# BurntSushi/rust-snappy

Hardware: NVIDIA H100
Metric: uncompressed GB/s, raw 64KB-block compress+decompress round trip (higher is better)
Workload: dtype u8

## Files before the change

### rust-snappy_b200/csrc/k2_decompress.cuh

```cuda
#pragma once
#include "common.cuh"

namespace sbk {

static const uint32_t K2_SMEM_PER_WARP = 256;

SB_DEVICE uint32_t k2_read_header(const uint8_t* in, uint32_t n, uint64_t* value) {
    uint64_t v = 0;
    unsigned shift = 0;
    for (uint32_t i = 0; i < n; i++) {
        if (shift >= 64) return 0;
        uint32_t b = in[i];
        if (b < 0x80) { *value = v | ((uint64_t)b << shift); return i + 1; }
        v |= (uint64_t)(b & 0x7F) << shift;
        shift += 7;
    }
    return 0;
}

template <bool kHeader = true>
SB_DEVICE uint32_t k2_decode_stream(const uint8_t* in, uint32_t n, uint8_t* dst, uint64_t cap,
                                    sb_error* st, uint32_t* out_len, uint32_t* elems) {
    const unsigned lane = lane_id();
    uint64_t dn64 = cap;
    uint32_t hl = 0;
    if constexpr (kHeader) {
        if (n == 0) { if (lane == 0) set_status(st, SB_EMPTY, 0, 0, 0); return SB_EMPTY; }
        dn64 = 0;
        hl = k2_read_header(in, n, &dn64);
        if (hl == 0) { if (lane == 0) set_status(st, SB_HEADER, 0, 0, 0); return SB_HEADER; }
        if (dn64 > kMaxInput) { if (lane == 0) set_status(st, SB_TOO_BIG, dn64, kMaxInput, 0); return SB_TOO_BIG; }
        if (dn64 > cap) { if (lane == 0) set_status(st, SB_BUFFER_TOO_SMALL, cap, dn64, 0); return SB_BUFFER_TOO_SMALL; }
    }

    const uint8_t* src = in + hl;
    const uint8_t* in_end = in + n;
    const uint32_t sn = n - hl, dn = (uint32_t)dn64;
    uint32_t s = 0, d = 0;

    while (s < sn) {
#include "k2_window.inc"
        const bool is_start = ((M >> lane) & 1u) && valid;
        const unsigned last = 31 - clz(M);

        uint32_t olen = (is_start && !spill) ? (uint32_t)len : 0u;
        uint32_t incl = olen;
#pragma unroll
        for (int k = 1; k < 32; k <<= 1) {
            const uint32_t t = shfl_up(incl, k);
            if (lane >= (unsigned)k) incl += t;
        }
        const uint32_t opos = incl - olen;
        const uint32_t win_out = shfl(incl, 31);
        const uint64_t de = (uint64_t)d + opos;
        const uint64_t sa = (uint64_t)s + lane + 1;

        const bool sure = (rem >= 40) && (dn - d >= win_out) &&
                          !any(is_start && (spill || (kind != 0 && (off == 0 || off > d + opos))));
        if (!sure) {
            uint32_t ecode = 0; uint64_t ea = 0, eb = 0, ec = 0;
            if (is_start) {
                if (kind == 0) {
                    uint64_t sp = sa;
                    if ((tag >> 2) >= 60) {
                        if (sa + 4 > sn) { ecode = SB_LITERAL; ea = 4; eb = sn - sa; ec = dn - de; }
                        sp = sa + (hdr - 1);
                    }
                    if (!ecode && (sn - sp < len || dn - de < len)) {
                        ecode = SB_LITERAL; ea = len; eb = sn - sp; ec = dn - de;
                    }
                } else {
                    const unsigned nb = hdr - 1;
                    if (sa + 4 > sn) {
                        if (nb == 1) { if (sa >= sn) { ecode = SB_COPY_READ; ea = 1; eb = sn - sa; } }
                        else if (nb == 2) { if (sa + 1 >= sn) { ecode = SB_COPY_READ; ea = 2; eb = sn - sa; } }
                        else { ecode = SB_COPY_READ; ea = 4; eb = sn - sa; }
                    }
                    if (!ecode && (off == 0 || de < off)) { ecode = SB_OFFSET; ea = off; eb = de; }
                    if (!ecode && de + len > dn) { ecode = SB_COPY_WRITE; ea = len; eb = dn - de; }
                }
            }
            const uint32_t emask = ballot(ecode != 0);
            if (emask) {
                const unsigned first = ffs(emask) - 1;
                if (lane == first) set_status(st, ecode, ea, eb, ec);
                return shfl(ecode, first);
            }
        }

        {
            const unsigned own = 31 - clz(M & (0xFFFFFFFFu >> (31 - lane)));
            const uint32_t pk = shfl((opos << 8) | (hdr << 4) | (kind << 1) | (spill ? 1u : 0u), own);
            const unsigned ohdr = (pk >> 4) & 0xFu;
            if (valid && (pk & 7u) == 0 && lane >= own + ohdr)
                dst[d + (pk >> 8) + (lane - own - ohdr)] = (uint8_t)tag;
        }
        syncwarp();

        {
            uint8_t* const wout = dst + d;
            const uint32_t cpk = opos | ((uint32_t)len << 12);
            const bool is_copy = is_start && kind != 0;
            const bool indep = is_copy && (uint32_t)len <= 32 && off >= opos + (uint32_t)len;
            const uint32_t im = ballot(indep);
            if (im) {
                const uint32_t ilen = indep ? (uint32_t)len : 0u;
                uint32_t cincl = ilen;
#pragma unroll
                for (int k = 1; k < 32; k <<= 1) {
                    const uint32_t t2 = shfl_up(cincl, k);
                    if (lane >= (unsigned)k) cincl += t2;
                }
                const uint32_t cpos = cincl - ilen, ctot = shfl(cincl, 31);
                if (indep) {
                    const uint32_t rk = popc(im & ((1u << lane) - 1u));
                    elems[rk * 2] = cpk | (cpos << 20);
                    elems[rk * 2 + 1] = off;
                }
                syncwarp();
                for (uint32_t base = 0; base < ctot; base += 64) {
                    uint32_t dsto[2], srco[2];
                    uint8_t v[2];
                    bool on[2];
#pragma unroll
                    for (int q = 0; q < 2; q++) {
                        const uint32_t lo = base + 32 * q;
                        const uint32_t bit = (indep && cpos >= lo && cpos < lo + 32) ? 1u << (cpos - lo) : 0u;
                        const uint32_t Bm = reduce_or(bit);
                        const uint32_t before = popc(ballot(indep && cpos < lo));
                        const uint32_t t = lo + lane;
                        on[q] = t < ctot;
                        const uint32_t rk = before + popc(Bm & (0xFFFFFFFFu >> (31 - lane))) - 1;
                        const uint32_t e0 = on[q] ? elems[rk * 2] : 0u, e1 = on[q] ? elems[rk * 2 + 1] : 0u;
                        dsto[q] = (e0 & 0xFFFu) + (t - (e0 >> 20));
                        srco[q] = e1;
                    }
#pragma unroll
                    for (int q = 0; q < 2; q++) v[q] = on[q] ? wout[(int64_t)dsto[q] - (int64_t)srco[q]] : (uint8_t)0;
#pragma unroll
                    for (int q = 0; q < 2; q++) if (on[q]) wout[dsto[q]] = v[q];
                }
            }
            syncwarp();
            uint32_t cm = ballot(is_copy && !indep);
            while (cm) {
                const unsigned j = ffs(cm) - 1;
                cm &= cm - 1;
                const uint32_t pk1 = shfl(cpk, j), coff = shfl(off, j);
                const uint32_t clen = pk1 >> 12;
                uint8_t* out = wout + (pk1 & 0xFFFu);
                if (coff >= clen || clen <= 32) {
                    if (lane < clen) out[lane] = out[(int64_t)(coff >= clen || lane < coff ? lane : lane % coff) - (int64_t)coff];
                    if (clen > 32 && lane + 32 < clen) out[lane + 32] = out[(int64_t)lane + 32 - (int64_t)coff];
                } else {
                    const uint8_t* from = out - coff;
                    for (uint32_t k = lane; k < clen; k += 32) out[k] = from[k % coff];
                }
                syncwarp();
            }
        }

        const uint32_t lpk = shfl((uint32_t)(spill ? 1u : 0u) | (hdr << 1), last);
        if (lpk & 1u) {
            const uint32_t llen = shfl((uint32_t)len, last);
            const uint32_t lsrc = s + last + (lpk >> 1);
            warp_copy(dst + d + win_out, src + lsrc, llen);
            syncwarp();
            s = lsrc + llen;
            d += win_out + llen;
        } else {
            s += shfl(E, 0);
            d += win_out;
        }
    }
    if (d != dn) {
        if (lane == 0) set_status(st, SB_HEADER_MISMATCH, dn, d, 0);
        return SB_HEADER_MISMATCH;
    }
    if (lane == 0) { set_status(st, SB_OK, 0, 0, 0); if (out_len) *out_len = (uint32_t)dn; }
    return SB_OK;
}

SB_DEVICE void k2_decompress_body(const BatchDesc& b) {
    const unsigned warps_per_block = block_dim() >> 5;
    uint32_t* elems = (uint32_t*)smem() + warp_id() * 64;
    const uint64_t nwarps = (uint64_t)grid_dim() * warps_per_block;
    for (uint64_t u = (uint64_t)block_idx() * warps_per_block + warp_id(); u < b.count; u += nwarps) {
        const uint32_t i = (uint32_t)u;
        if (b.out_lens && lane_id() == 0) b.out_lens[i] = 0;
        k2_decode_stream(unit_in(b, i), unit_in_len(b, i), unit_out(b, i), unit_out_cap(b, i),
                         b.statuses ? &b.statuses[i] : nullptr, b.out_lens ? &b.out_lens[i] : nullptr, elems);
    }
}

}
```

### rust-snappy_b200/csrc/k2_window.inc

```
const uintptr_t A = (uintptr_t)(src + s);
const unsigned mis = (unsigned)(A & 3u);
uint32_t word = 0;
if (lane < 10) {
    const uint8_t* wp = (const uint8_t*)(A - mis) + 4 * lane;
    if (wp >= in && wp + 4 <= in_end) {
        word = *(const uint32_t*)wp;
    } else {
        for (int k = 0; k < 4; k++)
            if (wp + k >= in && wp + k < in_end) word |= (uint32_t)wp[k] << (8 * k);
    }
}
const unsigned bi = mis + lane;
const uint32_t lo = shfl(word, bi >> 2), hi = shfl(word, (bi >> 2) + 1);
const unsigned sh = (bi & 3u) * 8;
const uint32_t tag = funnel_r(lo, hi, sh) & 0xFFu;
const uint32_t next4 = sh == 24 ? hi : funnel_r(lo, hi, sh + 8);
const uint32_t rem = sn - s;
const bool valid = lane < rem;

const unsigned kind = tag & 3u;
unsigned hdr;
uint64_t len;
uint32_t off = 0;
if (kind == 0) {
    const unsigned L = tag >> 2;
    if (L < 60) { hdr = 1; len = L + 1; }
    else {
        const unsigned nb = L - 59;
        hdr = 1 + nb;
        len = (uint64_t)(nb == 4 ? next4 : (next4 & ((1u << (8 * nb)) - 1))) + 1;
    }
} else if (kind == 1) {
    hdr = 2; len = 4 + ((tag >> 2) & 7u); off = ((tag >> 5) << 8) | (next4 & 0xFFu);
} else if (kind == 2) {
    hdr = 3; len = 1 + (tag >> 2); off = next4 & 0xFFFFu;
} else {
    hdr = 5; len = 1 + (tag >> 2); off = next4;
}
const bool spill = valid && kind == 0 && (uint64_t)lane + hdr + len > 32;
uint32_t E = !valid ? 64u : spill ? 64u : (uint32_t)(lane + hdr + (kind == 0 ? (uint32_t)len : 0u));

uint32_t M = 1u << lane;
#pragma unroll
for (int r = 0; r < 4; r++) {
    const uint32_t M2 = shfl(M, E & 31u), E2 = shfl(E, E & 31u);
    if (E < 32) { M |= M2; E = E2; }
}
M = shfl(M, 0);
```

### rust-snappy_b200/csrc/simt.h

```cpp
#pragma once
#include <stdint.h>
#include <stddef.h>

#if defined(SB_EMU)
#ifndef SB_EMU_PRIMITIVES
#error "SB_EMU builds must include tests/emu/simt_emu.h first (it defines the warp primitives)"
#endif
namespace sbk {
SB_DEVICE void prefetch_l2(const void*) {}
}
#else

#include <cuda_runtime.h>

#define SB_DEVICE __device__ __forceinline__
#define SB_DEVICE_NOINLINE __device__ __noinline__
#define SB_FULL 0xFFFFFFFFu

namespace sbk {

SB_DEVICE unsigned lane_id() { return threadIdx.x & 31u; }
SB_DEVICE unsigned warp_id() { return threadIdx.x >> 5; }
SB_DEVICE unsigned thread_idx() { return threadIdx.x; }
SB_DEVICE unsigned block_dim() { return blockDim.x; }
SB_DEVICE unsigned block_idx() { return blockIdx.x; }
SB_DEVICE unsigned grid_dim() { return gridDim.x; }

SB_DEVICE uint32_t shfl(uint32_t v, unsigned src) { return __shfl_sync(SB_FULL, v, src); }
SB_DEVICE int shfl(int v, unsigned src) { return __shfl_sync(SB_FULL, v, src); }
SB_DEVICE uint64_t shfl(uint64_t v, unsigned src) { return __shfl_sync(SB_FULL, v, src); }
SB_DEVICE uint32_t shfl_up(uint32_t v, unsigned d) { return __shfl_up_sync(SB_FULL, v, d); }
SB_DEVICE uint32_t shfl_down(uint32_t v, unsigned d) { return __shfl_down_sync(SB_FULL, v, d); }
SB_DEVICE uint32_t shfl_xor(uint32_t v, unsigned m) { return __shfl_xor_sync(SB_FULL, v, m); }
SB_DEVICE uint32_t ballot(bool p) { return __ballot_sync(SB_FULL, p); }
SB_DEVICE bool any(bool p) { return __any_sync(SB_FULL, p); }
SB_DEVICE bool all(bool p) { return __all_sync(SB_FULL, p); }
SB_DEVICE uint32_t match_any(uint32_t v) { return __match_any_sync(SB_FULL, v); }
SB_DEVICE void syncwarp() { __syncwarp(); }
SB_DEVICE void syncthreads() { __syncthreads(); }
SB_DEVICE void bar_sync(unsigned id, unsigned nthreads) {
    asm volatile("bar.sync %0, %1;" ::"r"(id), "r"(nthreads) : "memory");
}
SB_DEVICE void bar_arrive(unsigned id, unsigned nthreads) {
    asm volatile("bar.arrive %0, %1;" ::"r"(id), "r"(nthreads) : "memory");
}

SB_DEVICE int popc(uint32_t v) { return __popc(v); }
SB_DEVICE int ffs(uint32_t v) { return __ffs(v); }
SB_DEVICE int clz(uint32_t v) { return __clz(v); }
SB_DEVICE int ffsll(uint64_t v) { return __ffsll((long long)v); }
SB_DEVICE uint32_t funnel_r(uint32_t lo, uint32_t hi, unsigned sh) { return __funnelshift_r(lo, hi, sh); }
SB_DEVICE uint32_t byte_perm(uint32_t a, uint32_t b, uint32_t s) { return __byte_perm(a, b, s); }

SB_DEVICE uint32_t atomic_add(uint32_t* p, uint32_t v) { return atomicAdd(p, v); }
SB_DEVICE unsigned long long atomic_add(unsigned long long* p, unsigned long long v) { return atomicAdd(p, v); }
SB_DEVICE uint32_t atomic_min(uint32_t* p, uint32_t v) { return atomicMin(p, v); }
SB_DEVICE void threadfence() { __threadfence(); }
SB_DEVICE void threadfence_block() { __threadfence_block(); }
SB_DEVICE uint32_t reduce_or(uint32_t v) { return __reduce_or_sync(SB_FULL, v); }
SB_DEVICE uint32_t reduce_add(uint32_t v) { return __reduce_add_sync(SB_FULL, v); }
SB_DEVICE uint32_t reduce_max(uint32_t v) { return __reduce_max_sync(SB_FULL, v); }
SB_DEVICE void spin() { __nanosleep(32); }
SB_DEVICE void spin_long() { __nanosleep(1500); }
SB_DEVICE uint32_t ld_volatile(const uint32_t* p) { return *(const volatile uint32_t*)p; }
SB_DEVICE void st_volatile(uint32_t* p, uint32_t v) { *(volatile uint32_t*)p = v; }
SB_DEVICE uint64_t ld_volatile64(const uint64_t* p) { return *(const volatile uint64_t*)p; }
SB_DEVICE void prefetch_l2(const void* p) { asm volatile("prefetch.global.L2 [%0];" :: "l"(p)); }

SB_DEVICE uint32_t ldg32(const void* p) { return __ldg((const uint32_t*)p); }
SB_DEVICE uint4 ldg128(const void* p) { return __ldg((const uint4*)p); }
SB_DEVICE uint8_t ldg8(const void* p) { return __ldg((const uint8_t*)p); }
SB_DEVICE void stcs128(void* p, uint4 v) { __stcs((uint4*)p, v); }

SB_DEVICE void mbar_init(uint64_t* bar, unsigned count) {
    asm volatile("mbarrier.init.shared::cta.b64 [%0], %1;" ::"r"((uint32_t)__cvta_generic_to_shared(bar)), "r"(count) : "memory");
}
SB_DEVICE void mbar_arrive(uint64_t* bar) {
    asm volatile("mbarrier.arrive.shared::cta.b64 _, [%0];" ::"r"((uint32_t)__cvta_generic_to_shared(bar)) : "memory");
}
SB_DEVICE bool mbar_try_wait(uint64_t* bar, unsigned parity, unsigned hint_ns) {
    uint32_t done;
    asm volatile("{ .reg .pred p; mbarrier.try_wait.parity.shared::cta.b64 p, [%1], %2, %3; selp.u32 %0, 1, 0, p; }"
                 : "=r"(done) : "r"((uint32_t)__cvta_generic_to_shared(bar)), "r"(parity), "r"(hint_ns) : "memory");
    return done != 0;
}
SB_DEVICE void st8_stream(uint8_t* p, uint8_t v) { __stcs(p, v); }
extern __shared__ __align__(128) unsigned char sb_dyn_smem[];
SB_DEVICE unsigned char* smem() { return sb_dyn_smem; }

}
#endif
```

### rust-snappy_b200/csrc/snapb200.cu

```cuda
#include <cuda_runtime.h>

#include <atomic>
#include <cstdio>
#include <cstdlib>
#include <cstring>
#include <mutex>
#include <vector>
#include <sched.h>
#include <time.h>

#include "k1_compress.cuh"
#include "k2_decompress.cuh"
#include "k3_crc32c.cuh"
#include "k4_frame.cuh"
#include "k5_frame_decode.cuh"
#include "k7_frame_index.cuh"
#include "k8_raw_split.cuh"
#include "k9_raw_batch_compress.cuh"
#include "k10_frame_batch_encode.cuh"
#include "k11_frame_batch_decode.cuh"
#include "k12_frame_range_decode.cuh"
#include "k13_frame_table.cuh"
#include "k14_frame_table_batch.cuh"

namespace {

template <int NG>
__global__ void __launch_bounds__((7 + NG) * 64, 1)
k1_m7_kernel(sb_batch b, uint32_t flags, uint64_t* rings, uint16_t* gtables, uint32_t* work, uint32_t* crcs) {
    sbk::k1_compress_body_multi<7, NG>(b, flags, rings, gtables, work, crcs);
}
const int K1_MAX_NG = 7;
const size_t K1_M7_SMEM = sbk::k1_multi_smem(7, K1_MAX_NG);
__global__ void __launch_bounds__(128) k2_decompress_kernel(sb_batch b) { sbk::k2_decompress_body(b); }
__global__ void __launch_bounds__(256) k3_crc_kernel(sb_batch b) { sbk::k3_crc_body(b); }
__global__ void __launch_bounds__(256) k4_fill_lens_kernel(uint32_t* lens, uint64_t n, uint32_t nchunks) { sbk::k4_fill_lens_body(lens, n, nchunks); }
__global__ void __launch_bounds__(1024) k4_scan_local_kernel(sbk::FramePlan p) { sbk::k4_scan_local_body(p); }
__global__ void __launch_bounds__(1024) k4_scan_tiles_kernel(sbk::FramePlan p) { sbk::k4_scan_tiles_body(p); }
__global__ void __launch_bounds__(256) k4_gather_kernel(sbk::FramePlan p) { sbk::k4_gather_body(p); }
__global__ void __launch_bounds__(256) k5_parse_kernel(sbk::DecodePlan p) { sbk::k5_parse_body(p); }
__global__ void __launch_bounds__(32) k5_walk_kernel(sbk::DecodePlan p) { sbk::k5_walk_body(p); }
__global__ void __launch_bounds__(1024) k5_scan_local_kernel(sbk::DecodePlan p) { sbk::k5_scan_local_body(p); }
__global__ void __launch_bounds__(1024) k5_scan_tiles_kernel(sbk::DecodePlan p) { sbk::k5_scan_tiles_body(p); }
__global__ void __launch_bounds__(128) k5_decode_kernel(sbk::DecodePlan p) { sbk::k5_decode_body(p); }
__global__ void __launch_bounds__(32) k5_finish_kernel(sbk::DecodePlan p) { sbk::k5_finish_body(p); }
__global__ void __launch_bounds__(256) k6_generate_kernel(sbk::GenPlan g) { sbk::k6_generate_body(g); }
__global__ void __launch_bounds__(128) k7_survivors_kernel(sbk::IndexPlan p) { sbk::k7_survivors_body(p); }
__global__ void __launch_bounds__(sbk::K7_STITCH_THREADS) k7_stitch_kernel(sbk::IndexPlan p) { sbk::k7_stitch_body(p); }
__global__ void __launch_bounds__(128) k7_emit_kernel(sbk::IndexPlan p) { sbk::k7_emit_body(p); }
__global__ void __launch_bounds__(32) k8_header_kernel(sbk::RawPlan p) { sbk::k8_header_body(p); }
__global__ void __launch_bounds__(128) k8_chains_kernel(sbk::RawPlan p) { sbk::k8_chains_body(p); }
__global__ void __launch_bounds__(128) k8_merge_kernel(sbk::RawPlan p) { sbk::k8_merge_body(p); }
__global__ void __launch_bounds__(sbk::K8_STITCH_THREADS) k8_stitch_kernel(sbk::RawPlan p) { sbk::k8_stitch_body(p); }
__global__ void __launch_bounds__(128) k8_counts_kernel(sbk::RawPlan p) { sbk::k8_counts_body(p); }
__global__ void __launch_bounds__(1024) k8_scan_local_kernel(sbk::RawPlan p) { sbk::k8_scan_local_body(p); }
__global__ void __launch_bounds__(1024) k8_scan_tiles_kernel(sbk::RawPlan p) { sbk::k8_scan_tiles_body(p); }
__global__ void __launch_bounds__(128) k8_cuts_kernel(sbk::RawPlan p) { sbk::k8_cuts_body(p); }
__global__ void __launch_bounds__(128) k8_blocks_kernel(sbk::RawPlan p) { sbk::k8_blocks_body(p); }
__global__ void __launch_bounds__(32) k8_fallback_kernel(sbk::RawPlan p) { sbk::k8_fallback_body(p); }
__global__ void __launch_bounds__(1024) k8b_plan_kernel(sbk::RawBatchPlan q) { sbk::k8b_plan_body(q); }
__global__ void __launch_bounds__(1024) k8b_plan_tiles_kernel(sbk::RawBatchPlan q) { sbk::k8b_plan_tiles_body(q); }
__global__ void __launch_bounds__(128, 12) k8b_chains_kernel(sbk::RawBatchPlan q) { sbk::k8b_chains_body(q); }
__global__ void __launch_bounds__(128) k8b_merge_kernel(sbk::RawBatchPlan q) { sbk::k8b_merge_body(q); }
__global__ void __launch_bounds__(sbk::K8_STITCH_THREADS) k8b_stitch_kernel(sbk::RawBatchPlan q) { sbk::k8b_stitch_body(q); }
__global__ void __launch_bounds__(128) k8b_counts_kernel(sbk::RawBatchPlan q) { sbk::k8b_counts_body(q); }
__global__ void __launch_bounds__(1024) k8b_scan_local_kernel(sbk::RawBatchPlan q) { sbk::k8b_scan_local_body(q); }
__global__ void __launch_bounds__(1024) k8b_scan_tiles_kernel(sbk::RawBatchPlan q) { sbk::k8b_scan_tiles_body(q); }
__global__ void __launch_bounds__(128) k8b_cuts_kernel(sbk::RawBatchPlan q) { sbk::k8b_cuts_body(q); }
__global__ void __launch_bounds__(128) k8b_blocks_kernel(sbk::RawBatchPlan q) { sbk::k8b_blocks_body(q); }
__global__ void __launch_bounds__(128) k8b_finish_kernel(sbk::RawBatchPlan q) { sbk::k8b_finish_body(q); }
__global__ void __launch_bounds__(256) k9_plan_kernel(sbk::RawCompressPlan q) { sbk::k9_plan_body(q); }
__global__ void __launch_bounds__(1024) k9_scan_local_kernel(sbk::RawCompressPlan q) { sbk::k9_scan_local_body(q); }
__global__ void __launch_bounds__(1024) k9_scan_tiles_kernel(sbk::RawCompressPlan q) { sbk::k9_scan_tiles_body(q); }
__global__ void __launch_bounds__(256) k9_fill_kernel(sbk::RawCompressPlan q) { sbk::k9_fill_body(q); }
__global__ void __launch_bounds__(1024) k9_bscan_local_kernel(sbk::RawCompressPlan q) { sbk::k9_bscan_local_body(q); }
__global__ void __launch_bounds__(1024) k9_bscan_tiles_kernel(sbk::RawCompressPlan q) { sbk::k9_bscan_tiles_body(q); }
__global__ void __launch_bounds__(256) k9_gather_kernel(sbk::RawCompressPlan q) { sbk::k9_gather_body(q); }
__global__ void __launch_bounds__(256) k9_finish_kernel(sbk::RawCompressPlan q) { sbk::k9_finish_body(q); }
__global__ void __launch_bounds__(256) k10_plan_kernel(sbk::FrameBatchPlan q) { sbk::k10_plan_body(q); }
__global__ void __launch_bounds__(1024) k10_iscan_local_kernel(sbk::FrameBatchPlan q) { sbk::k10_iscan_local_body(q); }
__global__ void __launch_bounds__(1024) k10_iscan_tiles_kernel(sbk::FrameBatchPlan q) { sbk::k10_iscan_tiles_body(q); }
__global__ void __launch_bounds__(256) k10_fill_kernel(sbk::FrameBatchPlan q) { sbk::k10_fill_body(q); }
__global__ void __launch_bounds__(1024) k10_bscan_local_kernel(sbk::FrameBatchPlan q) { sbk::k10_bscan_local_body(q); }
__global__ void __launch_bounds__(256) k10_gather_kernel(sbk::FrameBatchPlan q) { sbk::k10_gather_body(q); }
__global__ void __launch_bounds__(256) k10_finish_kernel(sbk::FrameBatchPlan q) { sbk::k10_finish_body(q); }
__global__ void __launch_bounds__(1024) k11_plan_kernel(sbk::FrameDecodeBatchPlan q) { sbk::k11_plan_body(q); }
__global__ void __launch_bounds__(1024) k11_plan_tiles_kernel(sbk::FrameDecodeBatchPlan q) { sbk::k11_plan_tiles_body(q); }
__global__ void __launch_bounds__(128) k11_survivors_kernel(sbk::FrameDecodeBatchPlan q) { sbk::k11_survivors_body(q); }
__global__ void __launch_bounds__(sbk::K7_STITCH_THREADS) k11_stitch_kernel(sbk::FrameDecodeBatchPlan q) { sbk::k11_stitch_body(q); }
__global__ void __launch_bounds__(256) k11_link_kernel(sbk::FrameDecodeBatchPlan q) { sbk::k11_link_body(q); }
__global__ void __launch_bounds__(1024) k11_count_kernel(sbk::FrameDecodeBatchPlan q) { sbk::k11_count_body(q); }
__global__ void __launch_bounds__(1024) k11_range_tiles_kernel(sbk::FrameDecodeBatchPlan q) { sbk::k11_range_tiles_body(q); }
__global__ void __launch_bounds__(128) k11_emit_kernel(sbk::FrameDecodeBatchPlan q) { sbk::k11_emit_body(q); }
__global__ void __launch_bounds__(256) k11_parse_kernel(sbk::FrameDecodeBatchPlan q) { sbk::k11_parse_body(q); }
__global__ void __launch_bounds__(64) k11_fill_kernel(sbk::FrameDecodeBatchPlan q) { sbk::k11_fill_body(q); }
__global__ void __launch_bounds__(1024) k11_oscan_local_kernel(sbk::FrameDecodeBatchPlan q) { sbk::k11_oscan_local_body(q); }
__global__ void __launch_bounds__(1024) k11_oscan_tiles_kernel(sbk::FrameDecodeBatchPlan q) { sbk::k11_oscan_tiles_body(q); }
__global__ void __launch_bounds__(128) k11_decode_kernel(sbk::FrameDecodeBatchPlan q) { sbk::k11_decode_body(q); }
__global__ void __launch_bounds__(256) k11_finish_kernel(sbk::FrameDecodeBatchPlan q) { sbk::k11_finish_body(q); }
__global__ void __launch_bounds__(1024) k12_plan_kernel(sbk::RangePlan q) { sbk::k12_plan_body(q); }
__global__ void __launch_bounds__(1024) k12_plan_tiles_kernel(sbk::RangePlan q) { sbk::k12_plan_tiles_body(q); }
__global__ void __launch_bounds__(128, 4) k12_decode_kernel(sbk::RangePlan q) { sbk::k12_decode_body(q); }
__global__ void __launch_bounds__(256) k12_finish_kernel(sbk::RangePlan q) { sbk::k12_finish_body(q); }
__global__ void __launch_bounds__(256) k13_export_kernel(sbk::DecodePlan p, sbk::TableHead* t) { sbk::k13_export_body(p, t); }
__global__ void __launch_bounds__(1024) k13_plan_kernel(sbk::TablePlan q) { sbk::k13_plan_body(q); }
__global__ void __launch_bounds__(1024) k13_plan_tiles_kernel(sbk::TablePlan q) { sbk::k13_plan_tiles_body(q); }
__global__ void __launch_bounds__(128, 4) k13_decode_kernel(sbk::TablePlan q) { sbk::k13_decode_body(q); }
__global__ void __launch_bounds__(128) k13_finish_kernel(sbk::TablePlan q) { sbk::k13_finish_body(q); }
__global__ void __launch_bounds__(1024) k14_size_local_kernel(sbk::TableBatchPlan t) { sbk::k14_size_local_body(t); }
__global__ void __launch_bounds__(1024) k14_size_tiles_kernel(sbk::TableBatchPlan t) { sbk::k14_size_tiles_body(t); }
__global__ void __launch_bounds__(256) k14_export_kernel(sbk::TableBatchPlan t) { sbk::k14_export_body(t); }

std::atomic<uint64_t> g_launches{0};
std::atomic<uint64_t> g_allocs{0};
const int K2_DEFAULT_CTAS_PER_SM = 16;
const int K1_DEFAULT_NG = 0;

int fail(sb_error* e, uint32_t code, uint64_t a = 0, uint64_t b = 0, uint64_t c = 0) {
    if (e) { e->code = code; e->_pad = 0; e->a = a; e->b = b; e->c = c; }
    return (int)code;
}
void ok(sb_error* e) { if (e) { e->code = 0; e->_pad = 0; e->a = e->b = e->c = 0; } }

#define CK(call)                                                                   \
    do {                                                                           \
        cudaError_t _e = (call);                                                   \
        if (_e != cudaSuccess) {                                                   \
            if (getenv("SNAPB200_DEBUG"))                                          \
                fprintf(stderr, "snapb200: %s -> %s (%s:%d)\n", #call, cudaGetErrorString(_e), __FILE__, __LINE__); \
            return fail(err, (_e == cudaErrorNoDevice || _e == cudaErrorInsufficientDriver || \
                              _e == cudaErrorNoKernelImageForDevice) ? SB_E_NO_DEVICE : SB_E_CUDA, (uint64_t)_e); \
        }                                                                          \
    } while (0)

struct DevBuf {
    void* p = nullptr;
    size_t cap = 0;
    cudaError_t need(size_t n) {
        if (n <= cap) return cudaSuccess;
        if (p) { cudaError_t e = cudaFree(p); p = nullptr; cap = 0; if (e != cudaSuccess) return e; }
        size_t want = n + n / 8 + 4096;
        g_allocs++;
        cudaError_t e = cudaMalloc(&p, want);
        if (e != cudaSuccess) { e = cudaMalloc(&p, n); want = n; }
        if (e == cudaSuccess) cap = want;
        return e;
    }
    template <class T> T* as() { return (T*)p; }
};

struct Lane {
    cudaStream_t s_compute = nullptr, s_h2d = nullptr, s_d2h = nullptr;
    cudaEvent_t ev_in[2] = {nullptr, nullptr}, ev_k[2] = {nullptr, nullptr}, ev_out[2] = {nullptr, nullptr};
    DevBuf in[2], slots[2], compact[2], lens[2], status[2], ptrs_in[2], ptrs_out[2], caps[2], ws[2];
    void* pinned[5] = {nullptr, nullptr, nullptr, nullptr, nullptr};
    size_t pinned_cap[5] = {0, 0, 0, 0, 0};
    std::mutex mu;
};
struct Ctx {
    int dev = -1, sms = 0;
    std::atomic<bool> ready{false};
    DevBuf rings, gtables, work;
    cudaEvent_t k1_done = nullptr;
    std::mutex k1_mu;
    Lane lane[2];
};
const int LANE_ENC = 0, LANE_DEC = 1;
Ctx g_ctx[16];
std::mutex g_init_mu;

int init_ctx(Ctx& c, int dev, sb_error* err) {
    cudaDeviceProp prop;
    CK(cudaGetDeviceProperties(&prop, dev));
    c.dev = dev; c.sms = prop.multiProcessorCount;
    CK(cudaFuncSetAttribute(k1_m7_kernel<0>, cudaFuncAttributeMaxDynamicSharedMemorySize, (int)K1_M7_SMEM));
    CK(cudaFuncSetAttribute(k1_m7_kernel<5>, cudaFuncAttributeMaxDynamicSharedMemorySize, (int)K1_M7_SMEM));
    CK(cudaFuncSetAttribute(k1_m7_kernel<7>, cudaFuncAttributeMaxDynamicSharedMemorySize, (int)K1_M7_SMEM));
    CK(c.rings.need((size_t)c.sms * (7 + K1_MAX_NG) * sbk::K1_RING_GW * 8));
    CK(c.gtables.need((size_t)c.sms * K1_MAX_NG * sbk::K1_TABLE_BYTES));
    CK(c.work.need(256));
    g_allocs += 19;
    CK(cudaEventCreateWithFlags(&c.k1_done, cudaEventDisableTiming));
    for (Lane& l : c.lane) {
        for (int k = 0; k < 2; k++) {
            CK(cudaEventCreateWithFlags(&l.ev_in[k], cudaEventDisableTiming));
            CK(cudaEventCreateWithFlags(&l.ev_k[k], cudaEventDisableTiming));
            CK(cudaEventCreateWithFlags(&l.ev_out[k], cudaEventDisableTiming));
        }
        CK(cudaStreamCreateWithFlags(&l.s_compute, cudaStreamNonBlocking));
        CK(cudaStreamCreateWithFlags(&l.s_h2d, cudaStreamNonBlocking));
        CK(cudaStreamCreateWithFlags(&l.s_d2h, cudaStreamNonBlocking));
    }
    return 0;
}
void destroy_partial(Ctx& c) {
    if (c.k1_done) { cudaEventDestroy(c.k1_done); c.k1_done = nullptr; }
    for (Lane& l : c.lane) {
        for (int k = 0; k < 2; k++) {
            if (l.ev_in[k]) { cudaEventDestroy(l.ev_in[k]); l.ev_in[k] = nullptr; }
            if (l.ev_k[k]) { cudaEventDestroy(l.ev_k[k]); l.ev_k[k] = nullptr; }
            if (l.ev_out[k]) { cudaEventDestroy(l.ev_out[k]); l.ev_out[k] = nullptr; }
        }
        if (l.s_compute) { cudaStreamDestroy(l.s_compute); l.s_compute = nullptr; }
        if (l.s_h2d) { cudaStreamDestroy(l.s_h2d); l.s_h2d = nullptr; }
        if (l.s_d2h) { cudaStreamDestroy(l.s_d2h); l.s_d2h = nullptr; }
    }
}

int get_ctx(Ctx** out, sb_error* err) {
    int dev = 0;
    CK(cudaGetDevice(&dev));
    if (dev < 0 || dev >= 16) return fail(err, SB_E_NO_DEVICE);
    Ctx& c = g_ctx[dev];
    if (!c.ready.load(std::memory_order_acquire)) {
        std::lock_guard<std::mutex> lk(g_init_mu);
        if (!c.ready.load(std::memory_order_relaxed)) {
            const int rc = init_ctx(c, dev, err);
            if (rc) { destroy_partial(c); return rc; }
            c.ready.store(true, std::memory_order_release);
        }
    }
    *out = &c;
    return 0;
}

int need_pinned(Lane& c, int slot, size_t n, sb_error* err) {
    if (n <= c.pinned_cap[slot]) return 0;
    if (c.pinned[slot]) { CK(cudaFreeHost(c.pinned[slot])); c.pinned[slot] = nullptr; c.pinned_cap[slot] = 0; }
    n += n / 4 + 4096;
    g_allocs++;
    CK(cudaHostAlloc(&c.pinned[slot], n, cudaHostAllocDefault));
    c.pinned_cap[slot] = n;
    return 0;
}

int launch_k1(Ctx& c, const sb_batch& b, uint32_t flags, uint32_t* crcs, cudaStream_t st, sb_error* err) {
    if (b.count == 0) return 0;
    static const int ng_env = getenv("SNAPB200_K1_NG") ? atoi(getenv("SNAPB200_K1_NG")) : K1_DEFAULT_NG;
    const unsigned ng = ng_env < 0 ? 0 : ng_env > K1_MAX_NG ? K1_MAX_NG : (unsigned)ng_env;
    static const int cap_env = getenv("SNAPB200_K1_CHAINS") ? atoi(getenv("SNAPB200_K1_CHAINS")) : 0;
    const unsigned cap = cap_env > 0 && (unsigned)cap_env < 7 + ng ? (unsigned)cap_env : 7 + ng;
    unsigned chains = (unsigned)(((uint64_t)b.count + c.sms - 1) / c.sms);
    if (chains > cap) chains = cap;
    unsigned mg = (unsigned)c.sms;
    if (mg > b.count) mg = b.count;
    std::lock_guard<std::mutex> k1lk(c.k1_mu);
    CK(cudaStreamWaitEvent(st, c.k1_done, 0));
    CK(cudaMemsetAsync(c.work.p, 0, 4, st));
    uint64_t* rg = c.rings.as<uint64_t>(); uint16_t* gt = c.gtables.as<uint16_t>(); uint32_t* wk = c.work.as<uint32_t>();
    if (ng > 5) k1_m7_kernel<7><<<mg, chains * 64, K1_M7_SMEM, st>>>(b, flags, rg, gt, wk, crcs);
    else if (ng > 0) k1_m7_kernel<5><<<mg, chains * 64, K1_M7_SMEM, st>>>(b, flags, rg, gt, wk, crcs);
    else k1_m7_kernel<0><<<mg, chains * 64, K1_M7_SMEM, st>>>(b, flags, rg, gt, wk, crcs);
    CK(cudaGetLastError());
    CK(cudaEventRecord(c.k1_done, st));
    g_launches++;
    return 0;
}
int launch_k2(Ctx& c, const sb_batch& b, cudaStream_t st, sb_error* err) {
    if (b.count == 0) return 0;
    const unsigned wpb = 4;
    uint64_t blocks = ((uint64_t)b.count + wpb - 1) / wpb;
    static const int per_sm = getenv("SNAPB200_K2_CTAS") ? atoi(getenv("SNAPB200_K2_CTAS")) : K2_DEFAULT_CTAS_PER_SM;
    unsigned grid = (unsigned)(per_sm * c.sms);
    if (grid > blocks) grid = (unsigned)blocks;
    k2_decompress_kernel<<<grid, 32 * wpb, wpb * sbk::K2_SMEM_PER_WARP, st>>>(b);
    g_launches++;
    CK(cudaGetLastError());
    return 0;
}
int launch_k3(Ctx& c, const sb_batch& b, cudaStream_t st, sb_error* err) {
    if (b.count == 0) return 0;
    const unsigned wpb = 8;
    uint64_t blocks = ((uint64_t)b.count + wpb - 1) / wpb;
    unsigned grid = (unsigned)(8 * c.sms);
    if (grid > blocks) grid = (unsigned)blocks;
    k3_crc_kernel<<<grid, 32 * wpb, sbk::K3_TABLE_BYTES, st>>>(b);
    g_launches++;
    CK(cudaGetLastError());
    return 0;
}
int launch_assemble(Ctx& c, const sbk::FramePlan& p, cudaStream_t st, sb_error* err) {
    if (p.nchunks == 0) return 0;
    const unsigned ntiles = (p.nchunks + sbk::K4_TILE - 1) / sbk::K4_TILE;
    k4_scan_local_kernel<<<ntiles, sbk::K4_TILE, 32 * sizeof(uint32_t), st>>>(p);
    k4_scan_tiles_kernel<<<1, 1024, 1024 * sizeof(uint64_t), st>>>(p);
    uint64_t blocks = ((uint64_t)p.nchunks + 7) / 8;
    unsigned grid = (unsigned)(8 * c.sms);
    if (grid > blocks) grid = (unsigned)blocks;
    k4_gather_kernel<<<grid, 256, 0, st>>>(p);
    g_launches += 3;
    CK(cudaGetLastError());
    return 0;
}

size_t put_varint(uint8_t* dst, uint64_t v) {
    size_t i = 0;
    while (v >= 0x80) { dst[i++] = (uint8_t)v | 0x80; v >>= 7; }
    dst[i++] = (uint8_t)v;
    return i;
}
size_t get_varint(const uint8_t* p, size_t n, uint64_t* out) {
    uint64_t v = 0;
    unsigned shift = 0;
    for (size_t i = 0; i < n; i++) {
        if (shift >= 64) return 0;
        uint8_t b = p[i];
        if (b < 0x80) { *out = v | ((uint64_t)b << shift); return i + 1; }
        v |= (uint64_t)(b & 0x7F) << shift;
        shift += 7;
    }
    return 0;
}

const uint64_t SB_MAX_INPUT = 0xFFFFFFFFull;
const uint32_t SB_MAX_BLOCK = 65536;
const uint32_t SB_MAX_CBLOCK = 76490;

size_t align_up(size_t v, size_t a) { return (v + a - 1) / a * a; }

struct EncodeWs { uint8_t* slots; uint32_t *lens_in, *clens, *crcs; uint64_t *offs, *tiles; };
uint64_t encode_ws_bytes(uint64_t n) {
    const uint64_t nchunks = (n + SB_MAX_BLOCK - 1) / SB_MAX_BLOCK;
    return align_up(nchunks * (uint64_t)sbk::kSlotStride, 256) + 3 * align_up(nchunks * 4 + 4, 256) +
           align_up((nchunks + 1) * 8, 256) + align_up((nchunks / sbk::K4_TILE + 3) * 8, 256) + 256;
}
EncodeWs carve_encode_ws(void* scratch, uint64_t nchunks) {
    uint8_t* p = (uint8_t*)align_up((size_t)scratch, 256);
    EncodeWs w;
    w.slots = p; p += align_up(nchunks * (uint64_t)sbk::kSlotStride, 256);
    w.lens_in = (uint32_t*)p; p += align_up(nchunks * 4 + 4, 256);
    w.clens = (uint32_t*)p; p += align_up(nchunks * 4 + 4, 256);
    w.crcs = (uint32_t*)p; p += align_up(nchunks * 4 + 4, 256);
    w.offs = (uint64_t*)p; p += align_up((nchunks + 1) * 8, 256);
    w.tiles = (uint64_t*)p;
    return w;
}

int compress_stream_ws(Ctx& c, const uint8_t* d_in, uint64_t n, uint8_t* d_out, uint64_t cap, int frame, int ident,
                       uint64_t* d_chunk_offs, sb_frame_result* d_result, void* scratch, cudaStream_t st, sb_error* err) {
    const uint64_t nchunks64 = (n + SB_MAX_BLOCK - 1) / SB_MAX_BLOCK;
    if (nchunks64 > 0xFFFFFFFFull) return fail(err, SB_TOO_BIG, n, SB_MAX_INPUT);
    const uint32_t nchunks = (uint32_t)nchunks64;
    sbk::FramePlan p;
    memset(&p, 0, sizeof p);
    if (frame) { if (ident && n) { memcpy(p.head, "\xff\x06\x00\x00sNaPpY", 10); p.head_len = 10; } }
    else p.head_len = (uint32_t)put_varint(p.head, n);
    if (n == 0) {
        sb_frame_result r;
        memset(&r, 0, sizeof r);
        r.bytes = p.head_len;
        if (p.head_len > cap) { r.status.code = SB_BUFFER_TOO_SMALL; r.status.a = cap; r.status.b = p.head_len; r.bytes = 0; }
        else if (p.head_len) CK(cudaMemcpyAsync(d_out, p.head, p.head_len, cudaMemcpyHostToDevice, st));
        if (d_result) CK(cudaMemcpyAsync(d_result, &r, sizeof r, cudaMemcpyHostToDevice, st));
        if (d_chunk_offs) { const uint64_t z = p.head_len; CK(cudaMemcpyAsync(d_chunk_offs, &z, 8, cudaMemcpyHostToDevice, st)); }
        CK(cudaStreamSynchronize(st));
        return 0;
    }
    const EncodeWs w = carve_encode_ws(scratch, nchunks);
    k4_fill_lens_kernel<<<(nchunks + 255) / 256, 256, 0, st>>>(w.lens_in, n, nchunks);
    g_launches++;
    sb_batch b;
    memset(&b, 0, sizeof b);
    b.in_base = d_in; b.in_stride = SB_MAX_BLOCK; b.in_lens = w.lens_in;
    b.out_base = w.slots; b.out_stride = sbk::kSlotStride; b.out_cap_uniform = sbk::kSlotStride;
    b.out_lens = w.clens; b.count = nchunks;
    int rc = launch_k1(c, b, frame ? 1u : 0u, frame ? w.crcs : nullptr, st, err);
    if (rc) return rc;
    p.in = d_in; p.n = n; p.slots = w.slots; p.clens = w.clens; p.crcs = w.crcs; p.nchunks = nchunks;
    p.frame = frame ? 1u : 0u; p.offs = d_chunk_offs ? d_chunk_offs : w.offs; p.tiles = w.tiles;
    p.out = d_out; p.cap = cap; p.result = d_result;
    return launch_assemble(c, p, st, err);
}

struct DecodeWs { sbk::FChunk* chunks; uint64_t *ooff, *tiles; sb_error* statuses; sbk::DecodeCtl* ctl; };
uint64_t decode_ws_bytes(uint64_t max_chunks) {
    return align_up(max_chunks * sizeof(sbk::FChunk) + 64, 256) + align_up((max_chunks + 1) * 8, 256) +
           align_up((max_chunks / sbk::K4_TILE + 3) * 8, 256) + align_up(max_chunks * sizeof(sb_error) + 64, 256) + 512;
}
DecodeWs carve_decode_ws(void* scratch, uint64_t max_chunks) {
    uint8_t* p = (uint8_t*)align_up((size_t)scratch, 256);
    DecodeWs w;
    w.chunks = (sbk::FChunk*)p; p += align_up(max_chunks * sizeof(sbk::FChunk) + 64, 256);
    w.ooff = (uint64_t*)p; p += align_up((max_chunks + 1) * 8, 256);
    w.tiles = (uint64_t*)p; p += align_up((max_chunks / sbk::K4_TILE + 3) * 8, 256);
    w.statuses = (sb_error*)p; p += align_up(max_chunks * sizeof(sb_error) + 64, 256);
    w.ctl = (sbk::DecodeCtl*)p;
    return w;
}
sbk::DecodePlan make_decode_plan(const uint8_t* d_in, uint64_t n, uint8_t* d_out, uint64_t cap, const uint64_t* d_index,
                                 uint32_t index_n, int fragment, sb_frame_result* d_result, void* scratch, uint32_t max_chunks) {
    const DecodeWs w = carve_decode_ws(scratch, max_chunks);
    sbk::DecodePlan p;
    memset(&p, 0, sizeof p);
    p.in = d_in; p.n = n; p.index = d_index; p.index_n = d_index ? index_n : 0; p.fragment = fragment ? 1u : 0u;
    p.chunks = w.chunks; p.cap_chunks = max_chunks; p.ooff = w.ooff; p.tiles = w.tiles; p.statuses = w.statuses; p.ctl = w.ctl;
    p.out = d_out; p.cap = cap; p.result = d_result;
    if (!d_index) { p.index = w.ooff; p.index_count = &w.ctl->index_count; }
    return p;
}

uint64_t k7_want_seg() {
    static const long long env = getenv("SNAPB200_K7_SEG") ? atoll(getenv("SNAPB200_K7_SEG")) : 0;
    return env > 0 ? (uint64_t)env : sbk::K7_SEG_DEFAULT;
}
int launch_k7(Ctx& c, const sbk::IndexPlan& p, cudaStream_t st, sb_error* err) {
    k7_survivors_kernel<<<p.nseg ? (p.nseg + 3) / 4 : 1, 128, 0, st>>>(p);
    k7_stitch_kernel<<<1, sbk::K7_STITCH_THREADS, sbk::K7_STITCH_SMEM, st>>>(p);
    k7_emit_kernel<<<p.nseg ? (p.nseg + 127) / 128 : 1, 128, 0, st>>>(p);
    g_launches += 3;
    CK(cudaGetLastError());
    return 0;
}
uint64_t index_ws_segs(uint64_t n) { return n / sbk::K7_SEG_DEFAULT + 2; }
uint64_t index_ws_bytes(uint64_t n) {
    return align_up(index_ws_segs(n) * sizeof(sbk::K7Seg), 256) + align_up(index_ws_segs(n) * 12, 256) + 256;
}

int decode_index_phase(Ctx& c, const sbk::DecodePlan& p, cudaStream_t st, sb_error* err) {
// ... 1267 lines not shown
```

Baseline: 50.73.

## Branchless tag decode, L1 prefetch of source, sink error locals, raise K2 CTA count

Replaces the branchy per-lane Snappy tag decode with branchless arithmetic using packed lookup constants for header size, length and offset masks. Adds an L1 prefetch of the compressed stream 128 bytes ahead on each window iteration. Moves the error-path locals inside the slow branch. Raises the default decompress CTAs per SM from 16 to 128, which changes grid sizing and occupancy and may add scheduling overhead if the launch is not clamped.

Result: faster. 52.20 (median of 6 runs) (+2.9%).

```diff
diff --git a/rust-snappy_b200/csrc/k2_decompress.cuh b/rust-snappy_b200/csrc/k2_decompress.cuh
--- a/rust-snappy_b200/csrc/k2_decompress.cuh
+++ b/rust-snappy_b200/csrc/k2_decompress.cuh
@@ -39,6 +39,7 @@
     uint32_t s = 0, d = 0;
 
     while (s < sn) {
+        prefetch_l1(src + (sn - s > 128u ? s + 128u : sn - 1));
 #include "k2_window.inc"
         const bool is_start = ((M >> lane) & 1u) && valid;
         const unsigned last = 31 - clz(M);
@@ -52,12 +53,12 @@
         }
         const uint32_t opos = incl - olen;
         const uint32_t win_out = shfl(incl, 31);
-        const uint64_t de = (uint64_t)d + opos;
-        const uint64_t sa = (uint64_t)s + lane + 1;
 
         const bool sure = (rem >= 40) && (dn - d >= win_out) &&
                           !any(is_start && (spill || (kind != 0 && (off == 0 || off > d + opos))));
         if (!sure) {
+            const uint64_t de = (uint64_t)d + opos;
+            const uint64_t sa = (uint64_t)s + lane + 1;
             uint32_t ecode = 0; uint64_t ea = 0, eb = 0, ec = 0;
             if (is_start) {
                 if (kind == 0) {
diff --git a/rust-snappy_b200/csrc/k2_window.inc b/rust-snappy_b200/csrc/k2_window.inc
--- a/rust-snappy_b200/csrc/k2_window.inc
+++ b/rust-snappy_b200/csrc/k2_window.inc
@@ -19,26 +19,14 @@
 const bool valid = lane < rem;
 
 const unsigned kind = tag & 3u;
-unsigned hdr;
-uint64_t len;
-uint32_t off = 0;
-if (kind == 0) {
-    const unsigned L = tag >> 2;
-    if (L < 60) { hdr = 1; len = L + 1; }
-    else {
-        const unsigned nb = L - 59;
-        hdr = 1 + nb;
-        len = (uint64_t)(nb == 4 ? next4 : (next4 & ((1u << (8 * nb)) - 1))) + 1;
-    }
-} else if (kind == 1) {
-    hdr = 2; len = 4 + ((tag >> 2) & 7u); off = ((tag >> 5) << 8) | (next4 & 0xFFu);
-} else if (kind == 2) {
-    hdr = 3; len = 1 + (tag >> 2); off = next4 & 0xFFFFu;
-} else {
-    hdr = 5; len = 1 + (tag >> 2); off = next4;
-}
-const bool spill = valid && kind == 0 && (uint64_t)lane + hdr + len > 32;
-uint32_t E = !valid ? 64u : spill ? 64u : (uint32_t)(lane + hdr + (kind == 0 ? (uint32_t)len : 0u));
+const uint32_t L = tag >> 2;
+const uint32_t nb = (kind == 0 && L >= 60) ? L - 59 : 0u;
+const uint32_t lm1 = nb ? (next4 & (0xFFFFFFFFu >> ((32 - 8 * nb) & 31u))) : (kind == 1 ? 3 + (L & 7u) : L);
+const unsigned hdr = kind ? (0x5320u >> (4 * kind)) & 0xFu : 1 + nb;
+const uint64_t len = (uint64_t)lm1 + 1;
+const uint32_t off = (next4 & (0xFFFFFFFFu >> ((0x00101800u >> (8 * kind)) & 0xFFu))) | (kind == 1 ? (tag & 0xE0u) << 3 : 0u);
+const bool spill = valid && kind == 0 && lm1 >= (lane + hdr < 32u ? 32u - lane - hdr : 0u);
+uint32_t E = (!valid || spill) ? 64u : lane + hdr + (kind == 0 ? lm1 + 1 : 0u);
 
 uint32_t M = 1u << lane;
 #pragma unroll
diff --git a/rust-snappy_b200/csrc/simt.h b/rust-snappy_b200/csrc/simt.h
--- a/rust-snappy_b200/csrc/simt.h
+++ b/rust-snappy_b200/csrc/simt.h
@@ -8,6 +8,7 @@
 #endif
 namespace sbk {
 SB_DEVICE void prefetch_l2(const void*) {}
+SB_DEVICE void prefetch_l1(const void*) {}
 }
 #else
 
@@ -66,6 +67,7 @@
 SB_DEVICE void st_volatile(uint32_t* p, uint32_t v) { *(volatile uint32_t*)p = v; }
 SB_DEVICE uint64_t ld_volatile64(const uint64_t* p) { return *(const volatile uint64_t*)p; }
 SB_DEVICE void prefetch_l2(const void* p) { asm volatile("prefetch.global.L2 [%0];" :: "l"(p)); }
+SB_DEVICE void prefetch_l1(const void* p) { asm volatile("prefetch.global.L1 [%0];" :: "l"(p)); }
 
 SB_DEVICE uint32_t ldg32(const void* p) { return __ldg((const uint32_t*)p); }
 SB_DEVICE uint4 ldg128(const void* p) { return __ldg((const uint4*)p); }
diff --git a/rust-snappy_b200/csrc/snapb200.cu b/rust-snappy_b200/csrc/snapb200.cu
--- a/rust-snappy_b200/csrc/snapb200.cu
+++ b/rust-snappy_b200/csrc/snapb200.cu
@@ -113,7 +113,7 @@
 
 std::atomic<uint64_t> g_launches{0};
 std::atomic<uint64_t> g_allocs{0};
-const int K2_DEFAULT_CTAS_PER_SM = 16;
+const int K2_DEFAULT_CTAS_PER_SM = 128;
 const int K1_DEFAULT_NG = 0;
 
 int fail(sb_error* e, uint32_t code, uint64_t a = 0, uint64_t b = 0, uint64_t c = 0) {
```
